# vovach777/llcomp

Hardware: AMD Instinct MI355X
Metric: encode+decode MPix/s on 4K RGB8, bit-exact (higher is better)
Workload: dtype int32

## Files before the change

llcomp_amd/csrc/dec_rows_asm.hpp:

```cpp
#pragma once
#include <cstdint>

namespace llcomp_mi {

#define LD_E0L "v32"
#define LD_E0H "v33"
#define LD_E0 "v[32:33]"
#define LD_E5L "v34"
#define LD_E5H "v35"
#define LD_E5 "v[34:35]"
#define LD_E6L "v36"
#define LD_E6H "v37"
#define LD_E6 "v[36:37]"
#define LD_E7L "v38"
#define LD_E7H "v39"
#define LD_E7 "v[38:39]"
#define LD_E1L "v40"
#define LD_E1H "v41"
#define LD_E1 "v[40:41]"
#define LD_E2L "v42"
#define LD_E2H "v43"
#define LD_E2 "v[42:43]"
#define LD_E3L "v44"
#define LD_E3H "v45"
#define LD_E3 "v[44:45]"
#define LD_E4L "v48"
#define LD_E4H "v49"
#define LD_E4 "v[48:49]"
#define LD_WINL "v46"
#define LD_WIN "v[46:47]"
#define LD_PROD "v50"
#define LD_R1 "v51"
#define LD_DIFF "v52"
#define LD_OFF "v52"
#define LD_EX "v32"
#define LD_W "v33"
#define LD_RUN "v40"
#define LD_NX "v41"
#define LD_T "v42"
#define LD_SX "s[56:57]"
#define LD_SA "s[58:59]"
#define LD_SW "s[60:61]"
#define LD_SP "s[62:63]"
#define LD_S5 "s[64:65]"
#define LD_SU "s[66:67]"
#define LD_SD "s[68:69]"
#define LD_S1L "s[68:69]"
#define LD_SM "s[70:71]"
#define LD_S1 "s70"
#define LD_S2 "s71"

#define LD_SPLIT(EL)                                                                                                       \
    "v_mul_u32_u24_sdwa " LD_PROD ", " EL ", %[range] dst_sel:DWORD dst_unused:UNUSED_PAD src0_sel:BYTE_1 src1_sel:DWORD\n\t" \
    "v_lshrrev_b32_e32 " LD_R1 ", 8, " LD_PROD "\n\t"                                                                      \
    "v_sub_u32_e32 %[range], %[range], " LD_R1 "\n\t"
#define LD_REFILL(N)                                         \
    "v_cmp_gt_u32_e32 vcc, %[c100], %[range]\n\t"            \
    "s_and_saveexec_b64 " LD_SW ", vcc\n\t"                  \
    "s_cbranch_execz .Lrf" N "_%=\n\t"                       \
    "v_lshlrev_b32_e32 %[range], 8, %[range]\n\t"            \
    "v_perm_b32 %[low], %[low], %[w32], %[sel]\n\t"          \
    "v_lshrrev_b32_e32 %[w32], 8, %[w32]\n"                   \
    ".Lrf" N "_%=:\n\t"                                      \
    "s_mov_b64 exec, " LD_SW "\n\t"
#define LD_REFILL_R1(N)                                           \
    "v_cmp_gt_u32_e32 vcc, %[c100], " LD_R1 "\n\t"                \
    "s_and_saveexec_b64 " LD_SW ", vcc\n\t"                       \
    "s_cbranch_execz .Lrf" N "_%=\n\t"                            \
    "v_and_b32_e32 %[range], 0xffffff00, " LD_PROD "\n\t"         \
    "v_perm_b32 %[low], %[low], %[w32], %[sel]\n\t"               \
// ... 15 lines not shown
    "v_lshrrev_b32_e32 " LD_E1L ", 16, %[w0]\n\t"             \
    "v_and_b32_e32 " LD_E2L ", 0xffff, %[w1]\n\t"             \
    "v_lshrrev_b32_e32 " LD_E3L ", 16, %[w1]\n\t"             \
    "v_and_b32_e32 " LD_E4L ", 0xffff, %[w2]\n\t"             \
    "ds_read_b64 " LD_E1 ", " LD_E1L "\n\t"                   \
    "ds_read_b64 " LD_E2 ", " LD_E2L "\n\t"                   \
    "ds_read_b64 " LD_E3 ", " LD_E3L "\n\t"                   \
    "ds_read_b64 " LD_E4 ", " LD_E4L "\n\t"                   \
    "v_lshrrev_b32_e32 " LD_E5L ", 16, %[w2]\n\t"             \
    "v_and_b32_e32 " LD_E6L ", 0xffff, %[w3]\n\t"             \
    "v_lshrrev_b32_e32 " LD_E7L ", 16, %[w3]\n\t"             \
    "ds_read_b64 " LD_E5 ", " LD_E5L "\n\t"                   \
    "ds_read_b64 " LD_E6 ", " LD_E6L "\n\t"                   \
    "ds_read_b64 " LD_E7 ", " LD_E7L "\n\t"

__device__ __forceinline__ void dec_rows_sample_asm(uint32_t& low, uint32_t& range, unsigned long long& win, uint32_t w0, uint32_t w1,
                                                    uint32_t w2, uint32_t w3, uint32_t bank, uint32_t& hot, uint32_t& value, uint32_t& w32) {
    asm volatile(
        "s_mov_b64 " LD_SX ", exec\n\t"
        "v_and_b32_e32 %[w32], 0xffffff, " LD_WINL "\n\t"
        "v_or_b32_e32 %[w32], 0x1000000, %[w32]\n\t"
        "v_and_b32_e32 " LD_OFF ", 0xffff, %[w0]\n\t"
        "ds_read_b64 " LD_E0 ", " LD_OFF "\n\t"
        "v_mov_b32_e32 %[value], 0\n\t"
        "s_cmp_lg_u32 %[hot], 0\n\t"
        "s_cbranch_scc0 .Lcold_%=\n\t"
        LD_FETCH_REST
        "s_waitcnt lgkmcnt(7)\n\t"
        "s_branch .Lzero_%=\n"
        ".Lcold_%=:\n\t"
        "s_waitcnt lgkmcnt(0)\n"
        ".Lzero_%=:\n\t"
        LD_SPLIT(LD_E0L)
        "v_sub_co_u32_e32 " LD_DIFF ", vcc, %[low], %[range]\n\t"
        "ds_write_b16_d16_hi %[bank], " LD_E0L "\n\t"
        "s_and_b64 " LD_SA ", exec, vcc\n\t"
        "s_andn2_b64 exec, exec, vcc\n\t"
        "s_cbranch_execz .Lz1_%=\n\t"
        "v_mov_b32_e32 %[low], " LD_DIFF "\n\t"
        "v_mov_b32_e32 %[range], " LD_R1 "\n\t"
        "ds_write_b16_d16_hi %[bank], " LD_E0H "\n"
        ".Lz1_%=:\n\t"
        "s_mov_b64 exec, " LD_SX "\n\t"
        LD_REFILL("0")
        "s_and_b64 exec, " LD_SA ", " LD_SA "\n\t"
        "s_cbranch_execz .Ldone_%=\n\t"
        "s_cmp_lg_u32 %[hot], 0\n\t"
        "s_cbranch_scc1 .Lhave_%=\n\t"
        LD_FETCH_REST
        ".Lhave_%=:\n\t"
        "v_mov_b32_e32 " LD_EX ", 0\n\t"
        "v_mov_b32_e32 " LD_W ", 1\n\t"
        "s_waitcnt lgkmcnt(0)\n\t"
        "s_mov_b64 " LD_SM ", 0\n\t"
        LD_UNARY(LD_E1L, LD_E1H, "2", "1", "s_mov_b64 " LD_S1L ", exec\n\t")
        LD_UNARY(LD_E2L, LD_E2H, "256", "2", "s_mov_b64 " LD_SM ", exec\n\t")
        LD_UNARY(LD_E3L, LD_E3H, "258", "3", "")
        "s_mov_b64 " LD_SU ", exec\n\t"
        ".p2align 6\n"
        ".Lu_%=:\n\t"
        "s_waitcnt lgkmcnt(0)\n\t"
        LD_SPLIT(LD_E4L)
        "v_sub_co_u32_e32 %[low], vcc, %[low], %[range]\n\t"
        "s_andn2_b64 exec, exec, vcc\n\t"
        "s_cbranch_execz .Lu_done_%=\n\t"
        "v_lshrrev_b32_e32 " LD_OFF ", 16, " LD_E4H "\n\t"
        "ds_read_b64 " LD_E4 ", " LD_OFF "\n\t"
        "v_add_u32_e32 " LD_EX ", 1, " LD_EX "\n\t"
        "v_mov_b32_e32 %[range], " LD_R1 "\n\t"
        LD_REFILL_R1("4")
        "s_branch .Lu_%=\n"
        ".Lu_done_%=:\n\t"
        "s_mov_b64 exec, " LD_SU "\n\t"
        "ds_write_b16_d16_hi %[bank], " LD_E4L " offset:512\n"
        ".Lx_done_%=:\n\t"
        "s_mov_b64 exec, " LD_SA "\n\t"
        "v_add_u32_e32 %[low], %[low], %[range]\n\t"
        LD_REFILL("5")
        "v_cmp_lt_u32_e32 vcc, 31, " LD_EX "\n\t"
        "s_cbranch_vccz .Lexok_%=\n\t"
        "s_and_saveexec_b64 " LD_SP ", vcc\n\t"
        "v_mov_b32_e32 %[w32], 0\n\t"
        "s_andn2_b64 exec, " LD_SP ", exec\n\t"
        "s_cbranch_execz .Ldone_%=\n"
        ".Lexok_%=:\n\t"
        "s_mov_b64 " LD_S5 ", exec\n\t"
        "s_and_b64 exec, exec, " LD_S1L "\n\t"
        "s_cbranch_execz .Lvalue_%=\n\t"
        "s_mov_b64 " LD_SU ", exec\n\t"
        LD_SPLIT(LD_E5L)
        "v_sub_co_u32_e32 " LD_DIFF ", vcc, %[low], %[range]\n\t"
        "ds_write_b16_d16_hi %[bank], " LD_E5L " offset:514\n\t"
        "s_andn2_b64 " LD_SP ", exec, vcc\n\t"
        "v_addc_co_u32_e32 " LD_W ", vcc, " LD_W ", " LD_W ", vcc\n\t"
        "v_mov_b32_e32 " LD_RUN ", 0\n\t"
        "s_and_b64 exec, " LD_SP ", " LD_SP "\n\t"
        "s_cbranch_execz .Lp5_%=\n\t"
        "v_mov_b32_e32 %[low], " LD_DIFF "\n\t"
        "v_mov_b32_e32 %[range], " LD_R1 "\n\t"
        "ds_write_b16_d16_hi %[bank], " LD_E5H " offset:514\n"
        ".Lp5_%=:\n\t"
        "s_mov_b64 exec, " LD_SU "\n\t"
        LD_REFILL("6")
        "v_add_u32_e32 " LD_T ", -1, " LD_EX "\n\t"
        "s_and_b64 exec, exec, " LD_SM "\n\t"
        "s_cbranch_execz .Lm_skip_%=\n\t"
        "s_mov_b64 " LD_SP ", exec\n\t"
        "v_add_u32_e32 " LD_NX ", -2, " LD_EX "\n\t"
        "v_lshrrev_b32_e32 " LD_RUN ", " LD_NX ", %[sentv]\n\t"
        ".p2align 6\n"
        ".Lm_%=:\n\t"
        "s_waitcnt lgkmcnt(0)\n\t"
        LD_SPLIT(LD_E6L)
        "v_sub_co_u32_e32 " LD_DIFF ", vcc, %[low], %[range]\n\t"
        "s_nop 1\n\t"
        "v_cndmask_b32_e32 %[range], " LD_R1 ", %[range], vcc\n\t"
        "v_cndmask_b32_e32 %[low], " LD_DIFF ", %[low], vcc\n\t"
        "v_cndmask_b32_e32 " LD_NX ", " LD_E6H ", " LD_E6L ", vcc\n\t"
        "v_addc_co_u32_e32 " LD_RUN ", vcc, " LD_RUN ", " LD_RUN ", vcc\n\t"
        "s_mov_b64 " LD_SD ", vcc\n\t"
        "v_lshrrev_b32_e32 " LD_OFF ", 16, " LD_NX "\n\t"
        "ds_read_b64 " LD_E6 ", " LD_OFF "\n\t"
        "v_cmp_gt_u32_e32 vcc, %[c100], %[range]\n\t"
        "s_and_saveexec_b64 " LD_SW ", vcc\n\t"
        "s_cbranch_execz .Lmr_%=\n\t"
        "v_lshlrev_b32_e32 %[range], 8, %[range]\n\t"
        "v_perm_b32 %[low], %[low], %[w32], %[sel]\n\t"
        "v_lshrrev_b32_e32 %[w32], 8, %[w32]\n"
        ".Lmr_%=:\n\t"
        "s_andn2_b64 exec, " LD_SW ", " LD_SD "\n\t"
        "s_cbranch_execnz .Lm_%=\n\t"
        "s_mov_b64 exec, " LD_SP "\n\t"
        "ds_write_b16_d16_hi %[bank], " LD_NX " offset:768\n"
        ".Lm_skip_%=:\n\t"
        "s_mov_b64 exec, " LD_SU "\n\t"
        "v_lshlrev_b32_e32 " LD_W ", " LD_T ", " LD_W "\n\t"
        "v_or_b32_e32 " LD_W ", " LD_W ", " LD_RUN "\n"
        ".Lvalue_%=:\n\t"
        "s_mov_b64 exec, " LD_S5 "\n\t"
        "v_lshlrev_b32_e64 " LD_T ", " LD_EX ", 1\n\t"
        "v_add_u32_e32 " LD_T ", -1, " LD_T "\n\t"
        "v_xor_b32_e32 %[value], " LD_W ", " LD_T "\n\t"
        LD_SPLIT(LD_E7L)
        "v_sub_co_u32_e32 " LD_DIFF ", vcc, %[low], %[range]\n\t"
        "ds_write_b16_d16_hi %[bank], " LD_E7L " offset:770\n\t"
        "s_andn2_b64 exec, exec, vcc\n\t"
        "s_cbranch_execz .Lp7_%=\n\t"
        "v_mov_b32_e32 %[low], " LD_DIFF "\n\t"
        "v_mov_b32_e32 %[range], " LD_R1 "\n\t"
        "ds_write_b16_d16_hi %[bank], " LD_E7H " offset:770\n\t"
        "v_sub_u32_e32 %[value], 0, %[value]\n"
        ".Lp7_%=:\n\t"
        "s_mov_b64 exec, " LD_S5 "\n\t"
        LD_REFILL("7")
        ".Ldone_%=:\n\t"
        "s_mov_b64 exec, " LD_SX "\n\t"
        "v_ffbh_u32_e32 " LD_DIFF ", %[w32]\n\t"
        "v_add_u32_e32 " LD_DIFF ", -7, " LD_DIFF "\n\t"
        "v_lshrrev_b64 " LD_WIN ", " LD_DIFF ", " LD_WIN "\n\t"
        "s_bcnt1_i32_b64 " LD_S1 ", " LD_SA "\n\t"
        "s_bcnt1_i32_b64 " LD_S2 ", " LD_SX "\n\t"
        "s_lshl_b32 " LD_S1 ", " LD_S1 ", 1\n\t"
        "s_cmp_ge_u32 " LD_S1 ", " LD_S2 "\n\t"
        "s_cselect_b32 %[hot], 1, 0\n\t"
        "s_mov_b64 exec, " LD_SX "\n\t"
        : [low] "+v"(low), [range] "+v"(range), "+{v[46:47]}"(win), [hot] "+s"(hot), [value] "=&v"(value), [w32] "=&v"(w32)
        : [w0] "v"(w0), [w1] "v"(w1), [w2] "v"(w2), [w3] "v"(w3), [bank] "v"(bank), [c100] "s"(0x100u), [sel] "s"(0x06050400u),
          [sentv] "v"(0x80000000u)
        : "vcc", "scc", "memory", "v32", "v33", "v34", "v35", "v36", "v37", "v38", "v39", "v40", "v41", "v42", "v43", "v44", "v45",
          "v48", "v49", "v50", "v51", "v52", "s56", "s57", "s58", "s59", "s60", "s61", "s62", "s63", "s64", "s65", "s66",
          "s67", "s68", "s69", "s70", "s71");
}

}
```

llcomp_amd/csrc/slice_kernels.hip:

```cpp
#include <algorithm>

#include "device_common.hpp"
#include "kernels.hpp"

#ifndef LLMI_ASM_ENC
#define LLMI_ASM_ENC 1
#endif
#if LLMI_ASM_ENC
#include "enc_rows_asm.hpp"
#endif
#ifndef LLMI_ASM_DEC
#define LLMI_ASM_DEC 1
#endif
#if LLMI_ASM_DEC
#include "dec_rows_asm.hpp"
#endif

namespace llcomp_mi {

namespace {

#ifdef LLMI_CLOCK_PROBE
constexpr uint32_t kProbeSlots = 1u << 15;
__device__ unsigned long long g_probe[2][kProbeSlots][2];
// ... 539 lines not shown
                    return w;
                }
            }
            return load_sym(ofs);
        };
        uint32_t s0 = load_at(sofs, 0);
        sofs += sstep;
        uint32_t s1 = total > 1 ? load_at(sofs, 1) : 0;
        sofs += sstep;
        uint32_t bank_base = uint32_t(uintptr_t((lds_u8_ptr) reinterpret_cast<uint8_t*>(rowbank))) + threadIdx.x * 4;
        asm volatile("" : "+v"(bank_base));
#if LLMI_ASM_ENC
        EncRowsExtra xs{0u, 0u, 0u};
        unsigned long long low_range = e.low | ((unsigned long long)e.range << 32);
#endif
        auto code = [&](uint32_t sy, uint32_t i) {
            uint32_t bofs;
            int res;
            if constexpr (PX) {
                const uint32_t G = (sy >> 8) & 0xFF;
                const int sum = int(sy & 0xFF) + int((sy >> 16) & 0xFF) - 2 * int(G);
                const int t = (sum + int((uint32_t(sum) >> 31) * 3u)) >> 2;
                const int v = int(__builtin_amdgcn_ubfe(sy, psh, 8)) - int(G & msub) + (t & int(my));
                const int dq = (pL - pl) & int(i >= 2 ? large : 0u);
                const int sg = dq >> 31;
                const uint32_t aq = uint32_t((dq ^ sg) - sg);
                bofs = ((aq + 511u) & 0x200u) + ((aq + 508u) & 0x200u);
                res = ((v - pl) ^ sg) - sg;
                pL = pl;
                pl = v;
            } else if constexpr (sizeof(SYM) == 2) {
                bofs = (sy >> 3) & 0x600u;
                res = int(sy << 20) >> 20;
            } else {
                bofs = (((sy & 0xFFFF) * 109u) >> 7) & 0x600u;
                res = int(sy) >> 16;
            }
#if LLMI_ASM_ENC
            enc_rows_sample_asm(low_range, e.wp, xs, bank_base + bofs, res, e.base);
            if (__builtin_expect(xs.any_pend != 0, 0)) {
                xs.any_pend = 0;
                if (xs.pend) enc_carry_back_flushed(e);
                xs.pend = 0;
            }
#else
            uint32_t* bp = reinterpret_cast<uint32_t*>(reinterpret_cast<uint8_t*>(rowbank) + threadIdx.x * 4 + bofs);
            Bank bank{{bp[0], bp[64]}, reinterpret_cast<uint8_t*>(bp)};
            if (hot) enc_residual<true, true>(e, bank, tab, res); else enc_residual<false, true>(e, bank, tab, res);
            hot = __builtin_amdgcn_readfirstlane(2 * __popcll(__ballot(res != 0)) >= __popcll(__ballot(true)));
#endif
        };
        const uint32_t total0 = __builtin_amdgcn_readfirstlane(total);
        const bool same = __builtin_amdgcn_ballot_w64(total != total0) == 0;
        const uint32_t tail = PX ? rows_px_tail(g.c) : 2u;
        const uint32_t n_bulk = same && total0 > tail ? total0 - tail : 0;
        uint32_t i = 0;
        for (; i < n_bulk; ++i) {
            s0 = consume_here(s0);
            const uint32_t s2 = load_sym(sofs);
            sofs += sstep;
            if (e.wp >= e.base + 16) enc_flush16(e);
            code(s0, i);
            s0 = s1;
            s1 = s2;
        }
        for (; i < total; ++i) {
            s0 = consume_here(s0);
            const uint32_t s2 = i + 2 < total ? load_at(sofs, i + 2) : 0;
            sofs += sstep;
            if (e.wp >= e.base + 16) enc_flush16(e);
            code(s0, i);
            s0 = s1;
            s1 = s2;
        }
#if LLMI_ASM_ENC
        e.low = uint32_t(low_range);
        e.range = uint32_t(low_range >> 32);
#endif
    } else {
        uint64_t* banks;
        uint32_t bsh;
        if constexpr (LDSTAB) {
            banks = reinterpret_cast<uint64_t*>(dyn_lds);
            bsh = 0;
        } else {
            banks = states + ((size_t(id >> g.lane_shift) * kContexts) << g.lane_shift) + (id & ((1u << g.lane_shift) - 1));
            bsh = g.lane_shift;
        }
        uint32_t fk = 0;
// ... 214 lines not shown
            uint32_t limit = ones + 1;
            asm volatile("" : "+v"(limit));
            do {
                nx = dec_step_acc<CHECKED>(d, prob_of(cur), cur, w);
                cur = entry_at(tab, nx);
            } while (w < limit);
            dec_put_state<6, INLDS>(bank, nx);
        }
    }
    uint32_t v = w ^ ones;
    if (dec_once<7, CHECKED, INLDS>(d, bank, E)) v = 0u - v;
    out = v;
    return true;
}

template <bool INLDS>
__device__ __forceinline__ bool dec_sample(RangeDec& d, Bank& bank, const entry_t* tab, uint32_t& hot, bool replay_always,
                                           uint32_t& v) {
    const uint32_t s_low = d.low, s_range = d.range, s_b0 = bank.w[0], s_b1 = bank.w[1], s_b2 = bank.w[2], s_b3 = bank.w[3];
    const unsigned long long s_win = d.win;
    bool ok;
#if LLMI_ASM_DEC
    if constexpr (INLDS) {
        uint32_t left;
        dec_rows_sample_asm(d.low, d.range, d.win, bank.w[0], bank.w[1], bank.w[2], bank.w[3], lds_address(bank.lds), hot, v, left);
        ok = left != 0;
    } else
#endif
    {
        ok = hot ? dec_residual<true, false, INLDS>(d, bank, tab, v) : dec_residual<false, false, INLDS>(d, bank, tab, v);
        hot = 2 * __popcll(__ballot(v != 0)) >= __popcll(__ballot(true));
    }
    const bool ran_dry = (INLDS && LLMI_ASM_DEC != 0) ? false : d.win == 0;
    if (__builtin_expect(!ok || ran_dry || replay_always, 0)) {
        ++d.replays;
        d.low = s_low; d.range = s_range; d.win = s_win;
        bank.w[0] = s_b0; bank.w[1] = s_b1;
        if constexpr (INLDS) {
            bank.w[2] = s_b2; bank.w[3] = s_b3;
            reinterpret_cast<uint32_t*>(bank.lds)[0] = s_b0;
// ... 42 lines not shown
    RangeDec d;
    const uint32_t len = min(slice_len[id], g.slice_cap - 16);
    const uint32_t grp = __builtin_amdgcn_readfirstlane(id >> g.lane_shift);
    const uint32_t lane_in_group = id & ((1u << g.lane_shift) - 1);
    dec_open(d, reinterpret_cast<const uint32_t*>(units) + ((size_t(grp) * (g.slice_cap >> 2)) << g.lane_shift), lane_in_group,
             g.lane_shift, len);

    int16_t* p0 = rec + lane_order_index(g, id, 0);
    const ptrdiff_t GW = ptrdiff_t(1) << g.lane_shift;
    int16_t* const gbase = rec + ((size_t(grp) * g.slice_samples) << g.lane_shift);
    uint32_t hot = 0;
    LLMI_PROBE_START();

    if constexpr (ROWS) {
        for (uint32_t k = 0; k < 12; ++k) rowbank[k * 64 + threadIdx.x] = lds_address(tab) * 0x00010001u;
        int l[NCH], L[NCH];
#pragma unroll
        for (int k = 0; k < NCH; ++k) l[k] = L[k] = 128;
        int held_val = 0;
        uint32_t held_ofs = lane_in_group * 2, next_ofs = held_ofs, step_ofs = 2u << g.lane_shift;
        uint32_t large = small_model ? 0u : ~0u, first = ~0u;
        asm volatile("" : "+v"(large), "+v"(first), "+v"(step_ofs));
        uint8_t* const bank0 = reinterpret_cast<uint8_t*>(rowbank) + threadIdx.x * 4;
        bool bad = false;
        auto pixel = [&]() {
#pragma unroll
            for (int k = 0; k < NCH; ++k) {
                if (window_low(d)) dec_append(d);
                asm volatile("global_store_short %0, %1, %2" : : "v"(held_ofs), "v"(held_val), "s"(gbase) : "memory");
                const int lv = l[k];
                const int dq = (L[k] - lv) & int(large);
                int sg = dq >> 31;
                asm volatile("" : "+v"(sg));
                const uint32_t aq = uint32_t((dq ^ sg) - sg);
                uint32_t o1 = ((aq + 0x7FFFFFFFu) >> 21) & 0x400u, o2 = ((aq + 0x7FFFFFFCu) >> 21) & 0x400u;
                asm volatile("" : "+v"(o1), "+v"(o2));
                uint32_t* bp = reinterpret_cast<uint32_t*>(bank0 + (o1 + o2));
                Bank bank{{bp[0], bp[64], bp[128], bp[192]}, reinterpret_cast<uint8_t*>(bp)};
                uint32_t v = 0;
                if (!dec_sample<true>(d, bank, tab, hot, replay_always, v)) bad = true;
                v = (v ^ uint32_t(sg)) - uint32_t(sg);
                const int val = int(int16_t(uint32_t(lv) + v));
                held_val = val;
                held_ofs = next_ofs;
                next_ofs += step_ofs;
                L[k] = lv ^ ((lv ^ val) & int(first));
                l[k] = val;
            }
            first = 0;
        };
        const uint32_t sw0 = __builtin_amdgcn_readfirstlane(r.sw);
        const uint32_t n_bulk = __builtin_amdgcn_ballot_w64(r.sw != sw0) == 0 ? sw0 : 0;
        uint32_t x = 0;
        for (; x < n_bulk; ++x) pixel();
        for (; x < r.sw; ++x) pixel();
        if (bad) atomicOr(status, kStBadExponent);
        asm volatile("global_store_short %0, %1, %2" : : "v"(held_ofs), "v"(held_val), "s"(gbase) : "memory");
        publish_count(counters, kCtrDecReplays, d.replays);
    } else {
        uint64_t* banks;
        uint32_t bsh;
        if constexpr (LDSTAB) {
            banks = reinterpret_cast<uint64_t*>(dyn_lds);
            bsh = 0;
        } else {
            banks = states + ((size_t(id >> g.lane_shift) * kContexts) << g.lane_shift) + (id & ((1u << g.lane_shift) - 1));
            bsh = g.lane_shift;
        }
        if constexpr (NCH == 0) {
            const uint32_t nch = g.nch;
// ... 307 lines not shown
```

Baseline: 29400.

## Specialize single-channel row decoder with dual register-set asm and unrolled pairs

Turns the row-sample asm into a macro that produces two variants (A/B), each with separate input and output coder-state operands and its own window register pair. Consecutive samples can then alternate register sets without copy moves. For NCH==1 it adds a paired, unrolled loop for full 64-lane groups with the large model; this loop drops the per-sample mask and writes stores straight to computed offsets. The encoder gets a similar in-place pairing. The cost is more code and a more complex bulk/tail split, which risks edge-case bugs.

Measured after the change: 29610 (median of 4 runs). Within noise of the previous version (+0.7%).

```diff
diff --git a/llcomp_amd/csrc/dec_rows_asm.hpp b/llcomp_amd/csrc/dec_rows_asm.hpp
--- a/llcomp_amd/csrc/dec_rows_asm.hpp
+++ b/llcomp_amd/csrc/dec_rows_asm.hpp
@@ -27,8 +27,6 @@
 #define LD_E4L "v48"
 #define LD_E4H "v49"
 #define LD_E4 "v[48:49]"
-#define LD_WINL "v46"
-#define LD_WIN "v[46:47]"
 #define LD_PROD "v50"
 #define LD_R1 "v51"
 #define LD_DIFF "v52"
@@ -54,6 +52,10 @@
     "v_mul_u32_u24_sdwa " LD_PROD ", " EL ", %[range] dst_sel:DWORD dst_unused:UNUSED_PAD src0_sel:BYTE_1 src1_sel:DWORD\n\t" \
     "v_lshrrev_b32_e32 " LD_R1 ", 8, " LD_PROD "\n\t"                                                                      \
     "v_sub_u32_e32 %[range], %[range], " LD_R1 "\n\t"
+#define LD_SPLIT_IO(EL)                                                                                                       \
+    "v_mul_u32_u24_sdwa " LD_PROD ", " EL ", %[range_in] dst_sel:DWORD dst_unused:UNUSED_PAD src0_sel:BYTE_1 src1_sel:DWORD\n\t" \
+    "v_lshrrev_b32_e32 " LD_R1 ", 8, " LD_PROD "\n\t"                                                                         \
+    "v_sub_u32_e32 %[range], %[range_in], " LD_R1 "\n\t"
 #define LD_REFILL(N)                                         \
     "v_cmp_gt_u32_e32 vcc, %[c100], %[range]\n\t"            \
     "s_and_saveexec_b64 " LD_SW ", vcc\n\t"                  \
@@ -99,162 +101,177 @@
     "ds_read_b64 " LD_E6 ", " LD_E6L "\n\t"                   \
     "ds_read_b64 " LD_E7 ", " LD_E7L "\n\t"
 
-__device__ __forceinline__ void dec_rows_sample_asm(uint32_t& low, uint32_t& range, unsigned long long& win, uint32_t w0, uint32_t w1,
-                                                    uint32_t w2, uint32_t w3, uint32_t bank, uint32_t& hot, uint32_t& value, uint32_t& w32) {
-    asm volatile(
-        "s_mov_b64 " LD_SX ", exec\n\t"
-        "v_and_b32_e32 %[w32], 0xffffff, " LD_WINL "\n\t"
-        "v_or_b32_e32 %[w32], 0x1000000, %[w32]\n\t"
-        "v_and_b32_e32 " LD_OFF ", 0xffff, %[w0]\n\t"
-        "ds_read_b64 " LD_E0 ", " LD_OFF "\n\t"
-        "v_mov_b32_e32 %[value], 0\n\t"
-        "s_cmp_lg_u32 %[hot], 0\n\t"
-        "s_cbranch_scc0 .Lcold_%=\n\t"
-        LD_FETCH_REST
-        "s_waitcnt lgkmcnt(7)\n\t"
-        "s_branch .Lzero_%=\n"
-        ".Lcold_%=:\n\t"
-        "s_waitcnt lgkmcnt(0)\n"
-        ".Lzero_%=:\n\t"
-        LD_SPLIT(LD_E0L)
-        "v_sub_co_u32_e32 " LD_DIFF ", vcc, %[low], %[range]\n\t"
-        "ds_write_b16_d16_hi %[bank], " LD_E0L "\n\t"
-        "s_and_b64 " LD_SA ", exec, vcc\n\t"
-        "s_andn2_b64 exec, exec, vcc\n\t"
-        "s_cbranch_execz .Lz1_%=\n\t"
-        "v_mov_b32_e32 %[low], " LD_DIFF "\n\t"
-        "v_mov_b32_e32 %[range], " LD_R1 "\n\t"
-        "ds_write_b16_d16_hi %[bank], " LD_E0H "\n"
-        ".Lz1_%=:\n\t"
-        "s_mov_b64 exec, " LD_SX "\n\t"
-        LD_REFILL("0")
-        "s_and_b64 exec, " LD_SA ", " LD_SA "\n\t"
-        "s_cbranch_execz .Ldone_%=\n\t"
-        "s_cmp_lg_u32 %[hot], 0\n\t"
-        "s_cbranch_scc1 .Lhave_%=\n\t"
-        LD_FETCH_REST
-        ".Lhave_%=:\n\t"
-        "v_mov_b32_e32 " LD_EX ", 0\n\t"
-        "v_mov_b32_e32 " LD_W ", 1\n\t"
-        "s_waitcnt lgkmcnt(0)\n\t"
-        "s_mov_b64 " LD_SM ", 0\n\t"
-        LD_UNARY(LD_E1L, LD_E1H, "2", "1", "s_mov_b64 " LD_S1L ", exec\n\t")
-        LD_UNARY(LD_E2L, LD_E2H, "256", "2", "s_mov_b64 " LD_SM ", exec\n\t")
-        LD_UNARY(LD_E3L, LD_E3H, "258", "3", "")
-        "s_mov_b64 " LD_SU ", exec\n\t"
-        ".p2align 6\n"
-        ".Lu_%=:\n\t"
-        "s_waitcnt lgkmcnt(0)\n\t"
-        LD_SPLIT(LD_E4L)
-        "v_sub_co_u32_e32 %[low], vcc, %[low], %[range]\n\t"
-        "s_andn2_b64 exec, exec, vcc\n\t"
-        "s_cbranch_execz .Lu_done_%=\n\t"
-        "v_lshrrev_b32_e32 " LD_OFF ", 16, " LD_E4H "\n\t"
-        "ds_read_b64 " LD_E4 ", " LD_OFF "\n\t"
-        "v_add_u32_e32 " LD_EX ", 1, " LD_EX "\n\t"
-        "v_mov_b32_e32 %[range], " LD_R1 "\n\t"
-        LD_REFILL_R1("4")
-        "s_branch .Lu_%=\n"
-        ".Lu_done_%=:\n\t"
-        "s_mov_b64 exec, " LD_SU "\n\t"
-        "ds_write_b16_d16_hi %[bank], " LD_E4L " offset:512\n"
-        ".Lx_done_%=:\n\t"
-        "s_mov_b64 exec, " LD_SA "\n\t"
-        "v_add_u32_e32 %[low], %[low], %[range]\n\t"
-        LD_REFILL("5")
-        "v_cmp_lt_u32_e32 vcc, 31, " LD_EX "\n\t"
-        "s_cbranch_vccz .Lexok_%=\n\t"
-        "s_and_saveexec_b64 " LD_SP ", vcc\n\t"
-        "v_mov_b32_e32 %[w32], 0\n\t"
-        "s_andn2_b64 exec, " LD_SP ", exec\n\t"
-        "s_cbranch_execz .Ldone_%=\n"
-        ".Lexok_%=:\n\t"
-        "s_mov_b64 " LD_S5 ", exec\n\t"
-        "s_and_b64 exec, exec, " LD_S1L "\n\t"
-        "s_cbranch_execz .Lvalue_%=\n\t"
-        "s_mov_b64 " LD_SU ", exec\n\t"
-        LD_SPLIT(LD_E5L)
-        "v_sub_co_u32_e32 " LD_DIFF ", vcc, %[low], %[range]\n\t"
-        "ds_write_b16_d16_hi %[bank], " LD_E5L " offset:514\n\t"
-        "s_andn2_b64 " LD_SP ", exec, vcc\n\t"
-        "v_addc_co_u32_e32 " LD_W ", vcc, " LD_W ", " LD_W ", vcc\n\t"
-        "v_mov_b32_e32 " LD_RUN ", 0\n\t"
-        "s_and_b64 exec, " LD_SP ", " LD_SP "\n\t"
-        "s_cbranch_execz .Lp5_%=\n\t"
-        "v_mov_b32_e32 %[low], " LD_DIFF "\n\t"
-        "v_mov_b32_e32 %[range], " LD_R1 "\n\t"
-        "ds_write_b16_d16_hi %[bank], " LD_E5H " offset:514\n"
-        ".Lp5_%=:\n\t"
-        "s_mov_b64 exec, " LD_SU "\n\t"
-        LD_REFILL("6")
-        "v_add_u32_e32 " LD_T ", -1, " LD_EX "\n\t"
-        "s_and_b64 exec, exec, " LD_SM "\n\t"
-        "s_cbranch_execz .Lm_skip_%=\n\t"
-        "s_mov_b64 " LD_SP ", exec\n\t"
-        "v_add_u32_e32 " LD_NX ", -2, " LD_EX "\n\t"
-        "v_lshrrev_b32_e32 " LD_RUN ", " LD_NX ", %[sentv]\n\t"
-        ".p2align 6\n"
-        ".Lm_%=:\n\t"
-        "s_waitcnt lgkmcnt(0)\n\t"
-        LD_SPLIT(LD_E6L)
-        "v_sub_co_u32_e32 " LD_DIFF ", vcc, %[low], %[range]\n\t"
-        "s_nop 1\n\t"
-        "v_cndmask_b32_e32 %[range], " LD_R1 ", %[range], vcc\n\t"
-        "v_cndmask_b32_e32 %[low], " LD_DIFF ", %[low], vcc\n\t"
-        "v_cndmask_b32_e32 " LD_NX ", " LD_E6H ", " LD_E6L ", vcc\n\t"
-        "v_addc_co_u32_e32 " LD_RUN ", vcc, " LD_RUN ", " LD_RUN ", vcc\n\t"
-        "s_mov_b64 " LD_SD ", vcc\n\t"
-        "v_lshrrev_b32_e32 " LD_OFF ", 16, " LD_NX "\n\t"
-        "ds_read_b64 " LD_E6 ", " LD_OFF "\n\t"
-        "v_cmp_gt_u32_e32 vcc, %[c100], %[range]\n\t"
-        "s_and_saveexec_b64 " LD_SW ", vcc\n\t"
-        "s_cbranch_execz .Lmr_%=\n\t"
-        "v_lshlrev_b32_e32 %[range], 8, %[range]\n\t"
-        "v_perm_b32 %[low], %[low], %[w32], %[sel]\n\t"
-        "v_lshrrev_b32_e32 %[w32], 8, %[w32]\n"
-        ".Lmr_%=:\n\t"
-        "s_andn2_b64 exec, " LD_SW ", " LD_SD "\n\t"
-        "s_cbranch_execnz .Lm_%=\n\t"
-        "s_mov_b64 exec, " LD_SP "\n\t"
-        "ds_write_b16_d16_hi %[bank], " LD_NX " offset:768\n"
-        ".Lm_skip_%=:\n\t"
-        "s_mov_b64 exec, " LD_SU "\n\t"
-        "v_lshlrev_b32_e32 " LD_W ", " LD_T ", " LD_W "\n\t"
-        "v_or_b32_e32 " LD_W ", " LD_W ", " LD_RUN "\n"
-        ".Lvalue_%=:\n\t"
-        "s_mov_b64 exec, " LD_S5 "\n\t"
-        "v_lshlrev_b32_e64 " LD_T ", " LD_EX ", 1\n\t"
-        "v_add_u32_e32 " LD_T ", -1, " LD_T "\n\t"
-        "v_xor_b32_e32 %[value], " LD_W ", " LD_T "\n\t"
-        LD_SPLIT(LD_E7L)
-        "v_sub_co_u32_e32 " LD_DIFF ", vcc, %[low], %[range]\n\t"
-        "ds_write_b16_d16_hi %[bank], " LD_E7L " offset:770\n\t"
-        "s_andn2_b64 exec, exec, vcc\n\t"
-        "s_cbranch_execz .Lp7_%=\n\t"
-        "v_mov_b32_e32 %[low], " LD_DIFF "\n\t"
-        "v_mov_b32_e32 %[range], " LD_R1 "\n\t"
-        "ds_write_b16_d16_hi %[bank], " LD_E7H " offset:770\n\t"
-        "v_sub_u32_e32 %[value], 0, %[value]\n"
-        ".Lp7_%=:\n\t"
-        "s_mov_b64 exec, " LD_S5 "\n\t"
-        LD_REFILL("7")
-        ".Ldone_%=:\n\t"
-        "s_mov_b64 exec, " LD_SX "\n\t"
-        "v_ffbh_u32_e32 " LD_DIFF ", %[w32]\n\t"
-        "v_add_u32_e32 " LD_DIFF ", -7, " LD_DIFF "\n\t"
-        "v_lshrrev_b64 " LD_WIN ", " LD_DIFF ", " LD_WIN "\n\t"
-        "s_bcnt1_i32_b64 " LD_S1 ", " LD_SA "\n\t"
-        "s_bcnt1_i32_b64 " LD_S2 ", " LD_SX "\n\t"
-        "s_lshl_b32 " LD_S1 ", " LD_S1 ", 1\n\t"
-        "s_cmp_ge_u32 " LD_S1 ", " LD_S2 "\n\t"
-        "s_cselect_b32 %[hot], 1, 0\n\t"
-        "s_mov_b64 exec, " LD_SX "\n\t"
-        : [low] "+v"(low), [range] "+v"(range), "+{v[46:47]}"(win), [hot] "+s"(hot), [value] "=&v"(value), [w32] "=&v"(w32)
-        : [w0] "v"(w0), [w1] "v"(w1), [w2] "v"(w2), [w3] "v"(w3), [bank] "v"(bank), [c100] "s"(0x100u), [sel] "s"(0x06050400u),
-          [sentv] "v"(0x80000000u)
-        : "vcc", "scc", "memory", "v32", "v33", "v34", "v35", "v36", "v37", "v38", "v39", "v40", "v41", "v42", "v43", "v44", "v45",
-          "v48", "v49", "v50", "v51", "v52", "s56", "s57", "s58", "s59", "s60", "s61", "s62", "s63", "s64", "s65", "s66",
-          "s67", "s68", "s69", "s70", "s71");
+#define LLMI_DEC_ROWS_SAMPLE(NAME, WIN_IN_L, WIN_IN, WIN_OUT, WIN_IN_REG, WIN_OUT_REG)                                                               \
+    __device__ __forceinline__ void NAME(uint32_t low_in, uint32_t range_in, unsigned long long win_in, uint32_t& low, uint32_t& range,              \
+                                         unsigned long long& win, uint32_t w0, uint32_t w1, uint32_t w2, uint32_t w3, uint32_t bank,                 \
+                                         uint32_t& hot, uint32_t& value, uint32_t& w32) {                                                            \
+    asm volatile(                                                                                                                                    \
+        "s_mov_b64 " LD_SX ", exec\n\t"                                                                                                              \
+        "v_and_b32_e32 %[w32], 0xffffff, " WIN_IN_L "\n\t"                        \
+        "v_or_b32_e32 %[w32], 0x1000000, %[w32]\n\t"                                                                                                 \
+        "v_and_b32_e32 " LD_OFF ", 0xffff, %[w0]\n\t"                                                                                                \
+        "ds_read_b64 " LD_E0 ", " LD_OFF "\n\t"                                                                                                      \
+        "v_mov_b32_e32 %[value], 0\n\t"                                                                                                              \
+        "s_cmp_lg_u32 %[hot], 0\n\t"                                                                                                                 \
+        "s_cbranch_scc0 .Lcold_%=\n\t"                                                                                                               \
+        LD_FETCH_REST                                                                                                                                \
+        "s_waitcnt lgkmcnt(7)\n\t"                                                                                                                   \
+        "s_branch .Lzero_%=\n"                                                                                                                       \
+        ".Lcold_%=:\n\t"                                                                                                                             \
+        "s_waitcnt lgkmcnt(0)\n"                                                                                                                     \
+                                                          \
+        ".Lzero_%=:\n\t"                                                                                                                             \
+        LD_SPLIT_IO(LD_E0L)                                 \
+        "v_sub_co_u32_e32 %[low], vcc, %[low_in], %[range]\n\t"                   \
+        "ds_write_b16_d16_hi %[bank], " LD_E0L "\n\t"                                                                                                \
+        "s_and_b64 " LD_SA ", exec, vcc\n\t"                                                                                                         \
+        "s_andn2_b64 exec, exec, vcc\n\t"                                                                                                            \
+        "s_cbranch_execz .Lz1_%=\n\t"                                                                                                                \
+        "v_mov_b32_e32 %[range], " LD_R1 "\n\t"                                                                                                      \
+        "ds_write_b16_d16_hi %[bank], " LD_E0H "\n"                                                                                                  \
+        ".Lz1_%=:\n\t"                                                                                                                               \
+        "s_mov_b64 exec, " LD_SX "\n\t"                                                                                                              \
+        LD_REFILL("0")                                                                                                                               \
+        "s_and_b64 exec, " LD_SA ", " LD_SA "\n\t"                                                                                                   \
+        "s_cbranch_execz .Ldone_%=\n\t"                                                                                                              \
+                       \
+        "v_add_u32_e32 %[low], %[low], %[range]\n\t"                                                                                                 \
+        "s_cmp_lg_u32 %[hot], 0\n\t"                                                                                                                 \
+        "s_cbranch_scc1 .Lhave_%=\n\t"                                                                                                               \
+        LD_FETCH_REST                                                                                                                                \
+        ".Lhave_%=:\n\t"                                                                                                                             \
+        "v_mov_b32_e32 " LD_EX ", 0\n\t"                                                                                                             \
+        "v_mov_b32_e32 " LD_W ", 1\n\t"                                                                                                              \
+        "s_waitcnt lgkmcnt(0)\n\t"                                                                                                                   \
+                                                                             \
+                       \
+        "s_mov_b64 " LD_SM ", 0\n\t"                                                                                                                 \
+        LD_UNARY(LD_E1L, LD_E1H, "2", "1", "s_mov_b64 " LD_S1L ", exec\n\t")                                                                         \
+        LD_UNARY(LD_E2L, LD_E2H, "256", "2", "s_mov_b64 " LD_SM ", exec\n\t")                                                                        \
+        LD_UNARY(LD_E3L, LD_E3H, "258", "3", "")                                                                                                     \
+        "s_mov_b64 " LD_SU ", exec\n\t"                                                                                                              \
+        ".p2align 6\n"                                                                                                                               \
+        ".Lu_%=:\n\t"                                                                                                                                \
+        "s_waitcnt lgkmcnt(0)\n\t"                                                                                                                   \
+        LD_SPLIT(LD_E4L)                                                                                                                             \
+        "v_sub_co_u32_e32 %[low], vcc, %[low], %[range]\n\t"                                                                                         \
+        "s_andn2_b64 exec, exec, vcc\n\t"                                                                                                            \
+        "s_cbranch_execz .Lu_done_%=\n\t"                                                                                                            \
+        "v_lshrrev_b32_e32 " LD_OFF ", 16, " LD_E4H "\n\t"                                                                                           \
+        "ds_read_b64 " LD_E4 ", " LD_OFF "\n\t"                                                                                                      \
+        "v_add_u32_e32 " LD_EX ", 1, " LD_EX "\n\t"                                                                                                  \
+        "v_mov_b32_e32 %[range], " LD_R1 "\n\t"                                                                                                      \
+        LD_REFILL_R1("4")                                                                                                                            \
+        "s_branch .Lu_%=\n"                                                                                                                          \
+        ".Lu_done_%=:\n\t"                                                                                                                           \
+        "s_mov_b64 exec, " LD_SU "\n\t"                                                                                                              \
+        "ds_write_b16_d16_hi %[bank], " LD_E4L " offset:512\n"                                                \
+        ".Lx_done_%=:\n\t"                                                                                                                           \
+        "s_mov_b64 exec, " LD_SA "\n\t"                                                                                                              \
+        "v_add_u32_e32 %[low], %[low], %[range]\n\t"                                \
+        LD_REFILL("5")                                                                                      \
+                                                    \
+        "v_cmp_lt_u32_e32 vcc, 31, " LD_EX "\n\t"                                                                                                    \
+        "s_cbranch_vccz .Lexok_%=\n\t"                                                                                                               \
+        "s_and_saveexec_b64 " LD_SP ", vcc\n\t"                                                                                                      \
+        "v_mov_b32_e32 %[w32], 0\n\t"                      \
+        "s_andn2_b64 exec, " LD_SP ", exec\n\t"                                                                                                      \
+        "s_cbranch_execz .Ldone_%=\n"                                                                                                                \
+        ".Lexok_%=:\n\t"                                                                                                                             \
+        "s_mov_b64 " LD_S5 ", exec\n\t"                                                \
+                                                       \
+        "s_and_b64 exec, exec, " LD_S1L "\n\t"                                                                                     \
+        "s_cbranch_execz .Lvalue_%=\n\t"                                                                                                             \
+        "s_mov_b64 " LD_SU ", exec\n\t"                                                                                                              \
+        LD_SPLIT(LD_E5L)                                                                                                                             \
+        "v_sub_co_u32_e32 " LD_DIFF ", vcc, %[low], %[range]\n\t"                                                                                    \
+        "ds_write_b16_d16_hi %[bank], " LD_E5L " offset:514\n\t"                                                                                     \
+        "s_andn2_b64 " LD_SP ", exec, vcc\n\t"                                                                       \
+        "v_addc_co_u32_e32 " LD_W ", vcc, " LD_W ", " LD_W ", vcc\n\t"                                                           \
+        "v_mov_b32_e32 " LD_RUN ", 0\n\t"                                                                                                            \
+        "s_and_b64 exec, " LD_SP ", " LD_SP "\n\t"                                                                                                   \
+        "s_cbranch_execz .Lp5_%=\n\t"                                                                                                                \
+        "v_mov_b32_e32 %[low], " LD_DIFF "\n\t"                                                                                                      \
+        "v_mov_b32_e32 %[range], " LD_R1 "\n\t"                                                                                                      \
+        "ds_write_b16_d16_hi %[bank], " LD_E5H " offset:514\n"                                                                                       \
+        ".Lp5_%=:\n\t"                                                                                                                               \
+        "s_mov_b64 exec, " LD_SU "\n\t"                                                                                                              \
+        LD_REFILL("6")                                                                                                                               \
+                           \
+        "v_add_u32_e32 " LD_T ", -1, " LD_EX "\n\t"                                                                         \
+        "s_and_b64 exec, exec, " LD_SM "\n\t"                                                                                      \
+        "s_cbranch_execz .Lm_skip_%=\n\t"                                                                                                            \
+        "s_mov_b64 " LD_SP ", exec\n\t"                                                                                                              \
+        "v_add_u32_e32 " LD_NX ", -2, " LD_EX "\n\t"                                                                                                 \
+        "v_lshrrev_b32_e32 " LD_RUN ", " LD_NX ", %[sentv]\n\t"                                                            \
+        ".p2align 6\n"                                                                                                                               \
+        ".Lm_%=:\n\t"                                                                                                                                \
+        "s_waitcnt lgkmcnt(0)\n\t"                                                                                                                   \
+        LD_SPLIT(LD_E6L)                                                                                                                             \
+        "v_sub_co_u32_e32 " LD_DIFF ", vcc, %[low], %[range]\n\t"                                                                                    \
+        "s_nop 1\n\t"                                                               \
+        "v_cndmask_b32_e32 %[range], " LD_R1 ", %[range], vcc\n\t"                                                                                   \
+        "v_cndmask_b32_e32 %[low], " LD_DIFF ", %[low], vcc\n\t"                                                                                     \
+        "v_cndmask_b32_e32 " LD_NX ", " LD_E6H ", " LD_E6L ", vcc\n\t"                                                                               \
+        "v_addc_co_u32_e32 " LD_RUN ", vcc, " LD_RUN ", " LD_RUN ", vcc\n\t"   \
+        "s_mov_b64 " LD_SD ", vcc\n\t"                                                                                                               \
+        "v_lshrrev_b32_e32 " LD_OFF ", 16, " LD_NX "\n\t"                                                                                            \
+        "ds_read_b64 " LD_E6 ", " LD_OFF "\n\t"                                                                                                      \
+        "v_cmp_gt_u32_e32 vcc, %[c100], %[range]\n\t"                                                                                                \
+        "s_and_saveexec_b64 " LD_SW ", vcc\n\t"                                                                                                      \
+        "s_cbranch_execz .Lmr_%=\n\t"                                                                                                                \
+        "v_lshlrev_b32_e32 %[range], 8, %[range]\n\t"                                                                                                \
+        "v_perm_b32 %[low], %[low], %[w32], %[sel]\n\t"                                                                                              \
+        "v_lshrrev_b32_e32 %[w32], 8, %[w32]\n"                                                                                                      \
+        ".Lmr_%=:\n\t"                                                                                                                               \
+        "s_andn2_b64 exec, " LD_SW ", " LD_SD "\n\t"                                              \
+        "s_cbranch_execnz .Lm_%=\n\t"                                                                                                                \
+        "s_mov_b64 exec, " LD_SP "\n\t"                                                                                                              \
+        "ds_write_b16_d16_hi %[bank], " LD_NX " offset:768\n"                                          \
+        ".Lm_skip_%=:\n\t"                                                                                                                           \
+        "s_mov_b64 exec, " LD_SU "\n\t"                                                                                                              \
+        "v_lshlrev_b32_e32 " LD_W ", " LD_T ", " LD_W "\n\t"                      \
+        "v_or_b32_e32 " LD_W ", " LD_W ", " LD_RUN "\n"                                                                                              \
+                                                    \
+        ".Lvalue_%=:\n\t"                                                                                                                            \
+        "s_mov_b64 exec, " LD_S5 "\n\t"                                                                                                              \
+        "v_lshlrev_b32_e64 " LD_T ", " LD_EX ", 1\n\t"                                                                                               \
+        "v_add_u32_e32 " LD_T ", -1, " LD_T "\n\t"                                                                                                   \
+        "v_xor_b32_e32 %[value], " LD_W ", " LD_T "\n\t"                                                                                             \
+                                                                                                         \
+        LD_SPLIT(LD_E7L)                                                                                                                             \
+        "v_sub_co_u32_e32 " LD_DIFF ", vcc, %[low], %[range]\n\t"                                                                                    \
+        "ds_write_b16_d16_hi %[bank], " LD_E7L " offset:770\n\t"                                                                                     \
+        "s_andn2_b64 exec, exec, vcc\n\t"                                                                                                            \
+        "s_cbranch_execz .Lp7_%=\n\t"                                                                                                                \
+        "v_mov_b32_e32 %[low], " LD_DIFF "\n\t"                                                                                                      \
+        "v_mov_b32_e32 %[range], " LD_R1 "\n\t"                                                                                                      \
+        "ds_write_b16_d16_hi %[bank], " LD_E7H " offset:770\n\t"                                                                                     \
+        "v_sub_u32_e32 %[value], 0, %[value]\n"                                                                                                      \
+        ".Lp7_%=:\n\t"                                                                                                                               \
+        "s_mov_b64 exec, " LD_S5 "\n\t"                                                                                                              \
+        LD_REFILL("7")                                                                                                                               \
+        ".Ldone_%=:\n\t"                                                                                                                             \
+        "s_mov_b64 exec, " LD_SX "\n\t"                                                                                                              \
+        "v_ffbh_u32_e32 " LD_DIFF ", %[w32]\n\t"                                       \
+        "v_add_u32_e32 " LD_DIFF ", -7, " LD_DIFF "\n\t"           \
+        "v_lshrrev_b64 " WIN_OUT ", " LD_DIFF ", " WIN_IN "\n\t"                                                                                      \
+        "s_bcnt1_i32_b64 " LD_S1 ", " LD_SA "\n\t"                                                                                                   \
+        "s_bcnt1_i32_b64 " LD_S2 ", " LD_SX "\n\t"                                                                                                   \
+        "s_lshl_b32 " LD_S1 ", " LD_S1 ", 1\n\t"                                                                                                     \
+        "s_cmp_ge_u32 " LD_S1 ", " LD_S2 "\n\t"                                                                                                      \
+        "s_cselect_b32 %[hot], 1, 0\n\t"                                                                                                             \
+        "s_mov_b64 exec, " LD_SX "\n\t"                                                                                                              \
+        : [low] "=&v"(low), [range] "=&v"(range), "=&" WIN_OUT_REG(win), [hot] "+s"(hot), [value] "=&v"(value), [w32] "=&v"(w32)                          \
+        : [low_in] "v"(low_in), [range_in] "v"(range_in), WIN_IN_REG(win_in), [w0] "v"(w0), [w1] "v"(w1), [w2] "v"(w2), [w3] "v"(w3),   \
+          [bank] "v"(bank), [c100] "s"(0x100u), [sel] "s"(0x06050400u),                                                                              \
+          [sentv] "v"(0x80000000u)                                                                                                                   \
+        : "vcc", "scc", "memory", "v32", "v33", "v34", "v35", "v36", "v37", "v38", "v39", "v40", "v41", "v42", "v43", "v44", "v45",                  \
+          "v48", "v49", "v50", "v51", "v52", "s56", "s57", "s58", "s59", "s60", "s61", "s62", "s63", "s64", "s65", "s66",                            \
+          "s67", "s68", "s69", "s70", "s71");                                                                                                        \
 }
 
+LLMI_DEC_ROWS_SAMPLE(dec_rows_sample_asm_a, "v46", "v[46:47]", "v[54:55]", "{v[46:47]}", "{v[54:55]}")
+LLMI_DEC_ROWS_SAMPLE(dec_rows_sample_asm_b, "v54", "v[54:55]", "v[46:47]", "{v[54:55]}", "{v[46:47]}")
+
 }
diff --git a/llcomp_amd/csrc/slice_kernels.hip b/llcomp_amd/csrc/slice_kernels.hip
--- a/llcomp_amd/csrc/slice_kernels.hip
+++ b/llcomp_amd/csrc/slice_kernels.hip
@@ -1,4 +1,5 @@
 #include <algorithm>
+#include <type_traits>
 
 #include "device_common.hpp"
 #include "kernels.hpp"
@@ -577,21 +578,20 @@
         EncRowsExtra xs{0u, 0u, 0u};
         unsigned long long low_range = e.low | ((unsigned long long)e.range << 32);
 #endif
-        auto code = [&](uint32_t sy, uint32_t i) {
-            uint32_t bofs;
-            int res;
+        [[maybe_unused]] uint32_t qmask = 0;
+        auto model = [&](uint32_t sy, auto plain, [[maybe_unused]] int& cl, [[maybe_unused]] int& cL, uint32_t& bofs, int& res) {
             if constexpr (PX) {
+                int dq = cL - cl;
+                if constexpr (!decltype(plain)::value) dq &= int(qmask);
+                const int sg = dq >> 31;
+                const uint32_t aq = uint32_t((dq ^ sg) - sg);
+                bofs = ((aq + 511u) & 0x200u) + ((aq + 508u) & 0x200u);
                 const uint32_t G = (sy >> 8) & 0xFF;
                 const int sum = int(sy & 0xFF) + int((sy >> 16) & 0xFF) - 2 * int(G);
                 const int t = (sum + int((uint32_t(sum) >> 31) * 3u)) >> 2;
                 const int v = int(__builtin_amdgcn_ubfe(sy, psh, 8)) - int(G & msub) + (t & int(my));
-                const int dq = (pL - pl) & int(i >= 2 ? large : 0u);
-                const int sg = dq >> 31;
-                const uint32_t aq = uint32_t((dq ^ sg) - sg);
-                bofs = ((aq + 511u) & 0x200u) + ((aq + 508u) & 0x200u);
-                res = ((v - pl) ^ sg) - sg;
-                pL = pl;
-                pl = v;
+                res = ((v - cl) ^ sg) - sg;
+                cL = v;
             } else if constexpr (sizeof(SYM) == 2) {
                 bofs = (sy >> 3) & 0x600u;
                 res = int(sy << 20) >> 20;
@@ -599,43 +599,100 @@
                 bofs = (((sy & 0xFFFF) * 109u) >> 7) & 0x600u;
                 res = int(sy) >> 16;
             }
+        };
+        auto bins = [&](uint32_t baddr, int res) {
 #if LLMI_ASM_ENC
-            enc_rows_sample_asm(low_range, e.wp, xs, bank_base + bofs, res, e.base);
+            enc_rows_sample_asm(low_range, e.wp, xs, baddr, res, e.base);
             if (__builtin_expect(xs.any_pend != 0, 0)) {
                 xs.any_pend = 0;
                 if (xs.pend) enc_carry_back_flushed(e);
                 xs.pend = 0;
             }
 #else
-            uint32_t* bp = reinterpret_cast<uint32_t*>(reinterpret_cast<uint8_t*>(rowbank) + threadIdx.x * 4 + bofs);
+            uint32_t* bp = reinterpret_cast<uint32_t*>(reinterpret_cast<uint8_t*>(rowbank) + threadIdx.x * 4 + (baddr - bank_base));
             Bank bank{{bp[0], bp[64]}, reinterpret_cast<uint8_t*>(bp)};
             if (hot) enc_residual<true, true>(e, bank, tab, res); else enc_residual<false, true>(e, bank, tab, res);
             hot = __builtin_amdgcn_readfirstlane(2 * __popcll(__ballot(res != 0)) >= __popcll(__ballot(true)));
 #endif
+        };
+        auto code = [&](uint32_t sy, auto plain, int& cl, int& cL) {
+            uint32_t bofs;
+            int res;
+            model(sy, plain, cl, cL, bofs, res);
+            bins(bank_base + bofs, res);
         };
         const uint32_t total0 = __builtin_amdgcn_readfirstlane(total);
         const bool same = __builtin_amdgcn_ballot_w64(total != total0) == 0;
         const uint32_t tail = PX ? rows_px_tail(g.c) : 2u;
         const uint32_t n_bulk = same && total0 > tail ? total0 - tail : 0;
-        uint32_t i = 0;
-        for (; i < n_bulk; ++i) {
+        constexpr std::false_type kMasked{};
+        constexpr std::true_type kPlain{};
+        auto tested = [&](uint32_t k) {
             s0 = consume_here(s0);
-            const uint32_t s2 = load_sym(sofs);
+            const uint32_t s2 = k + 2 < total ? load_at(sofs, k + 2) : 0;
             sofs += sstep;
             if (e.wp >= e.base + 16) enc_flush16(e);
-            code(s0, i);
+            code(s0, kMasked, pl, pL);
+            const int t = pl;
+            pl = pL;
+            pL = t;
             s0 = s1;
             s1 = s2;
-        }
-        for (; i < total; ++i) {
-            s0 = consume_here(s0);
-            const uint32_t s2 = i + 2 < total ? load_at(sofs, i + 2) : 0;
-            sofs += sstep;
-            if (e.wp >= e.base + 16) enc_flush16(e);
-            code(s0, i);
+        };
+#define LLMI_ROWS_SAMPLE(S, PLAIN, CL, CLL)                                                                      \
+        {                                                                                                        \
+            const uint32_t sc = consume_here(S);                                     \
+            S = load_sym(sofs);                                                                                  \
+            sofs += sstep;                                                                                       \
+            if (e.wp >= e.base + 16) enc_flush16(e);  \
+            code(sc, PLAIN, CL, CLL);                                                                            \
+        }
+#define LLMI_ROWS_SAMPLE_INPLACE(S, PLAIN, CL, CLL)                                                              \
+        {                                                                                                        \
+            S = consume_here(S);                                                                                 \
+            uint32_t bofs;                                                                                       \
+            int res;                                                                                             \
+            model(S, PLAIN, CL, CLL, bofs, res);                                                                 \
+            uint32_t baddr = bank_base + bofs;                                                                   \
+            asm volatile("" : "+v"(baddr), "+v"(res) : : "memory");           \
+            S = load_sym(sofs);                                                                                  \
+            sofs += sstep;                                                                                       \
+            if (e.wp >= e.base + 16) enc_flush16(e);                                                             \
+            bins(baddr, res);                                                                                    \
+        }
+        uint32_t i = 0;
+        if constexpr (PX) {
+            uint32_t n_peel = min(total, 2u);
+            asm volatile("" : "+v"(n_peel));
+            for (uint32_t k = 0; k < n_peel; ++k) tested(k);
+#if LLMI_ASM_ENC
+            xs.hot = __builtin_amdgcn_readfirstlane(xs.hot);
+            xs.any_pend = 0;
+#else
+            hot = __builtin_amdgcn_readfirstlane(hot);
+#endif
+            i = 2;
+            qmask = large;
+            asm volatile("" : "+v"(qmask));
+            if (!(g.flags & kGeoSmallModel)) {
+                for (; i + 2 <= n_bulk; i += 2) {
+                    LLMI_ROWS_SAMPLE_INPLACE(s0, kPlain, pl, pL)
+                    LLMI_ROWS_SAMPLE_INPLACE(s1, kPlain, pL, pl)
+                }
+            }
+        }
+        for (; i < n_bulk; ++i) {
+            LLMI_ROWS_SAMPLE(s0, kMasked, pl, pL)
+            const int t = pl;
+            pl = pL;
+            pL = t;
+            const uint32_t t0 = s0;
             s0 = s1;
-            s1 = s2;
-        }
+            s1 = t0;
+        }
+#undef LLMI_ROWS_SAMPLE
+#undef LLMI_ROWS_SAMPLE_INPLACE
+        for (; i < total; ++i) tested(i);
 #if LLMI_ASM_ENC
         e.low = uint32_t(low_range);
         e.range = uint32_t(low_range >> 32);
@@ -880,7 +937,7 @@
     return true;
 }
 
-template <bool INLDS>
+template <bool INLDS, bool SETB = false>
 __device__ __forceinline__ bool dec_sample(RangeDec& d, Bank& bank, const entry_t* tab, uint32_t& hot, bool replay_always,
                                            uint32_t& v) {
     const uint32_t s_low = d.low, s_range = d.range, s_b0 = bank.w[0], s_b1 = bank.w[1], s_b2 = bank.w[2], s_b3 = bank.w[3];
@@ -888,8 +945,15 @@
     bool ok;
 #if LLMI_ASM_DEC
     if constexpr (INLDS) {
-        uint32_t left;
-        dec_rows_sample_asm(d.low, d.range, d.win, bank.w[0], bank.w[1], bank.w[2], bank.w[3], lds_address(bank.lds), hot, v, left);
+        uint32_t left, n_low, n_range;
+        unsigned long long n_win;
+        if constexpr (SETB)
+            dec_rows_sample_asm_b(d.low, d.range, d.win, n_low, n_range, n_win, bank.w[0], bank.w[1], bank.w[2], bank.w[3],
+                                  lds_address(bank.lds), hot, v, left);
+        else
+            dec_rows_sample_asm_a(d.low, d.range, d.win, n_low, n_range, n_win, bank.w[0], bank.w[1], bank.w[2], bank.w[3],
+                                  lds_address(bank.lds), hot, v, left);
+        d.low = n_low; d.range = n_range; d.win = n_win;
         ok = left != 0;
     } else
 #endif
@@ -962,22 +1026,22 @@
 
     if constexpr (ROWS) {
         for (uint32_t k = 0; k < 12; ++k) rowbank[k * 64 + threadIdx.x] = lds_address(tab) * 0x00010001u;
-        int l[NCH], L[NCH];
-#pragma unroll
-        for (int k = 0; k < NCH; ++k) l[k] = L[k] = 128;
         int held_val = 0;
         uint32_t held_ofs = lane_in_group * 2, next_ofs = held_ofs, step_ofs = 2u << g.lane_shift;
-        uint32_t large = small_model ? 0u : ~0u, first = ~0u;
-        asm volatile("" : "+v"(large), "+v"(first), "+v"(step_ofs));
+        bool bad = false;
         uint8_t* const bank0 = reinterpret_cast<uint8_t*>(rowbank) + threadIdx.x * 4;
-        bool bad = false;
-        auto pixel = [&]() {
-#pragma unroll
-            for (int k = 0; k < NCH; ++k) {
+        if constexpr (NCH == 1 && LLMI_ASM_DEC != 0) {
+            asm volatile("" : "+v"(step_ofs));
+            int pl = 128, pL = 128;
+            auto sample = [&](auto setb, auto large_wide, uint32_t mask) {
                 if (window_low(d)) dec_append(d);
-                asm volatile("global_store_short %0, %1, %2" : : "v"(held_ofs), "v"(held_val), "s"(gbase) : "memory");
-                const int lv = l[k];
-                const int dq = (L[k] - lv) & int(large);
+                if constexpr (decltype(large_wide)::value) {
+                    asm volatile("global_store_short %0, %1, %2 offset:-128" : : "v"(next_ofs), "v"(pl), "s"(gbase) : "memory");
+                } else {
+                    asm volatile("global_store_short %0, %1, %2" : : "v"(held_ofs), "v"(pl), "s"(gbase) : "memory");
+                }
+                int dq = pL - pl;
+                if constexpr (!decltype(large_wide)::value) dq &= int(mask);
                 int sg = dq >> 31;
                 asm volatile("" : "+v"(sg));
                 const uint32_t aq = uint32_t((dq ^ sg) - sg);
@@ -986,22 +1050,79 @@
                 uint32_t* bp = reinterpret_cast<uint32_t*>(bank0 + (o1 + o2));
                 Bank bank{{bp[0], bp[64], bp[128], bp[192]}, reinterpret_cast<uint8_t*>(bp)};
                 uint32_t v = 0;
-                if (!dec_sample<true>(d, bank, tab, hot, replay_always, v)) bad = true;
+                if (!dec_sample<true, decltype(setb)::value>(d, bank, tab, hot, replay_always, v)) bad = true;
                 v = (v ^ uint32_t(sg)) - uint32_t(sg);
-                const int val = int(int16_t(uint32_t(lv) + v));
-                held_val = val;
-                held_ofs = next_ofs;
+                const int val = int(int16_t(uint32_t(pl) + v));
+                if constexpr (!decltype(large_wide)::value) held_ofs = next_ofs;
                 next_ofs += step_ofs;
-                L[k] = lv ^ ((lv ^ val) & int(first));
-                l[k] = val;
-            }
-            first = 0;
-        };
-        const uint32_t sw0 = __builtin_amdgcn_readfirstlane(r.sw);
-        const uint32_t n_bulk = __builtin_amdgcn_ballot_w64(r.sw != sw0) == 0 ? sw0 : 0;
-        uint32_t x = 0;
-        for (; x < n_bulk; ++x) pixel();
-        for (; x < r.sw; ++x) pixel();
+                pL = pl;
+                pl = val;
+            };
+            constexpr std::false_type kSetA{}, kGeneral{};
+            constexpr std::true_type kSetB{}, kLargeWide{};
+            const uint32_t large = small_model ? 0u : ~0u;
+            uint32_t mask = 0;
+            const uint32_t sw0 = __builtin_amdgcn_readfirstlane(r.sw);
+            const bool same = __builtin_amdgcn_ballot_w64(r.sw != sw0) == 0;
+            const bool pairs = same && g.lane_shift == 6 && !small_model;
+            const uint32_t n_single = same ? (pairs ? min(sw0, 2u) : sw0) : 0u;
+            uint32_t x = 0;
+            for (; x < n_single; ++x) {
+                sample(kSetA, kGeneral, mask);
+                mask = x >= 1 ? large : 0u;
+                asm volatile("" : "+v"(mask));
+            }
+            if (pairs && sw0 >= 4) {
+                for (; x + 2 <= sw0; x += 2) {
+                    sample(kSetA, kLargeWide, 0u);
+                    sample(kSetB, kLargeWide, 0u);
+                }
+                held_ofs = next_ofs - step_ofs;
+            }
+            for (; x < r.sw; ++x) {
+                sample(kSetA, kGeneral, mask);
+                mask = x >= 1 ? large : 0u;
+                asm volatile("" : "+v"(mask));
+            }
+            held_val = pl;
+        } else {
+            int l[NCH], L[NCH];
+#pragma unroll
+            for (int k = 0; k < NCH; ++k) l[k] = L[k] = 128;
+            uint32_t large = small_model ? 0u : ~0u, first = ~0u;
+            asm volatile("" : "+v"(large), "+v"(first), "+v"(step_ofs));
+            auto pixel = [&]() {
+#pragma unroll
+                for (int k = 0; k < NCH; ++k) {
+                    if (window_low(d)) dec_append(d);
+                    asm volatile("global_store_short %0, %1, %2" : : "v"(held_ofs), "v"(held_val), "s"(gbase) : "memory");
+                    const int lv = l[k];
+                    const int dq = (L[k] - lv) & int(large);
+                    int sg = dq >> 31;
+                    asm volatile("" : "+v"(sg));
+                    const uint32_t aq = uint32_t((dq ^ sg) - sg);
+                    uint32_t o1 = ((aq + 0x7FFFFFFFu) >> 21) & 0x400u, o2 = ((aq + 0x7FFFFFFCu) >> 21) & 0x400u;
+                    asm volatile("" : "+v"(o1), "+v"(o2));
+                    uint32_t* bp = reinterpret_cast<uint32_t*>(bank0 + (o1 + o2));
+                    Bank bank{{bp[0], bp[64], bp[128], bp[192]}, reinterpret_cast<uint8_t*>(bp)};
+                    uint32_t v = 0;
+                    if (!dec_sample<true>(d, bank, tab, hot, replay_always, v)) bad = true;
+                    v = (v ^ uint32_t(sg)) - uint32_t(sg);
+                    const int val = int(int16_t(uint32_t(lv) + v));
+                    held_val = val;
+                    held_ofs = next_ofs;
+                    next_ofs += step_ofs;
+                    L[k] = lv ^ ((lv ^ val) & int(first));
+                    l[k] = val;
+                }
+                first = 0;
+            };
+            const uint32_t sw0 = __builtin_amdgcn_readfirstlane(r.sw);
+            const uint32_t n_bulk = __builtin_amdgcn_ballot_w64(r.sw != sw0) == 0 ? sw0 : 0;
+            uint32_t x = 0;
+            for (; x < n_bulk; ++x) pixel();
+            for (; x < r.sw; ++x) pixel();
+        }
         if (bad) atomicOr(status, kStBadExponent);
         asm volatile("global_store_short %0, %1, %2" : : "v"(held_ofs), "v"(held_val), "s"(gbase) : "memory");
         publish_count(counters, kCtrDecReplays, d.replays);
```
